# AndreasKing-Goks/ast-sac

Hardware: AMD Instinct MI355X
Metric: batched env-steps/sec (two-ship AST) (higher is better)
Workload: dtype f64

## Files before the change

### ast_sac_amd/build_hash.py

```python
import hashlib
import os

_HERE = os.path.dirname(os.path.abspath(__file__))
_ROOT = os.path.dirname(_HERE)

SOURCES = {
    "shipsim": ["ast_sac_amd/csrc/shipsim_kernels.hip", "ast_sac_amd/csrc/shipsim_c2_pipe.hip",
                "ast_sac_amd/csrc/shipsim_types.hpp", "ast_sac_amd/csrc/shipsim_device.hpp",
                "ast_sac_amd/csrc/shipsim_state.hpp", "ast_sac_amd/csrc/shipsim_sbmpc.hpp",
                "ast_sac_amd/csrc/shipsim_diag.hpp", "ast_sac_amd/csrc/shipsim_config_host.hpp",
                "ast_sac_amd/csrc/shipsim_weather_host.hpp", "ast_sac_amd/csrc/shipsim_launch_host.hpp",
                "ast_sac_amd/csrc/shipsim_state_host.hpp", "include/shipsim.h",
                "ast_sac_amd/csrc/shipsim_resample.hip", "ast_sac_amd/csrc/shipsim_resample_host.hpp",
                "ast_sac_amd/csrc/shipsim_archive.hip", "ast_sac_amd/csrc/shipsim_archive_host.hpp",
                "ast_sac_amd/csrc/shipsim_grouping_host.hpp", "ast_sac_amd/csrc/shipsim_sbmpc_nominal.hpp",
                "ast_sac_amd/csrc/shipsim_tree.hip", "ast_sac_amd/csrc/shipsim_tree_host.hpp",
                "ast_sac_amd/csrc/shipsim_weather.hip"],
    "sacfused": ["ast_sac_amd/csrc/sac_kernels.hip", "include/sac_fused.h"],
}


HIPFLAGS = ["-O3", "--offload-arch=gfx950", "-ffp-contract=off", "-fPIC", "-shared", "-std=c++17"]
LIB_FLAGS = {"shipsim": ["-mllvm", "-amdgpu-sched-strategy=max-ilp", "-mllvm", "-amdgpu-use-amdgpu-trackers"],
             "sacfused": []}
OBJECTS = {"sacfused": [("ast_sac_amd/csrc/sac_kernels.hip", ["-DSACF_TU=1", "-mllvm", "-amdgpu-sched-strategy=max-ilp"]),
                        ("ast_sac_amd/csrc/sac_kernels.hip", ["-DSACF_TU=2"])],
           "shipsim": [("ast_sac_amd/csrc/shipsim_kernels.hip", ["-mllvm", "-disable-machine-licm"]),
                       ("ast_sac_amd/csrc/shipsim_c2_pipe.hip", []),
                       ("ast_sac_amd/csrc/shipsim_resample.hip", []),
                       ("ast_sac_amd/csrc/shipsim_archive.hip", []),
                       ("ast_sac_amd/csrc/shipsim_tree.hip", []),
                       ("ast_sac_amd/csrc/shipsim_weather.hip", [])]}


def lib_objects(lib):
    return [(src, LIB_FLAGS[lib] + extra) for src, extra in OBJECTS[lib]]


def lib_flag_sets(lib):
    return [flags for _, flags in lib_objects(lib)]
# ... 18 lines not shown
```

### ast_sac_amd/csrc/shipsim_device.hpp

```cpp
#pragma once
#include <hip/hip_runtime.h>
#include <stdint.h>

#include <type_traits>

#include "shipsim.h"
#include "shipsim_diag.hpp"
#include "shipsim_types.hpp"

namespace shipsim {

__device__ __forceinline__ double div_rcp(double d) {
  double r = __builtin_amdgcn_rcp(d);
  r = fma(r, fma(-d, r, 1.0), r);
  return fma(r, fma(-d, r, 1.0), r);
}
__device__ __forceinline__ double div_by(double n, double d, double y) {
  const double q0 = n * y;
  const double rem = fma(-d, q0, n);
  return __builtin_amdgcn_div_fixup(fma(rem, y, q0), d, n);
}

struct LaneWeather {
  double vc_n, vc_e, wind_speed, wind_sin, wind_cos;
};
constexpr int kWeatherCols = 5;
enum { WX_WIND_SPEED = 0, WX_WIND_SIN = 1, WX_WIND_COS = 2, WX_VC_N = 3, WX_VC_E = 4 };

struct AccI {
  int32_t a;
  __device__ __forceinline__ void set(int32_t x) { asm("v_accvgpr_write_b32 %0, %1" : "=a"(a) : "v"(x)); }
// ... 87 lines not shown

template <int CTRL>
__device__ __forceinline__ double dpp_d(double x) {
  int lo = __double2loint(x), hi = __double2hiint(x);
  lo = __builtin_amdgcn_mov_dpp(lo, CTRL, 0xF, 0xF, false);
  hi = __builtin_amdgcn_mov_dpp(hi, CTRL, 0xF, 0xF, false);
  return __hiloint2double(hi, lo);
}
template <int CTRL>
__device__ __forceinline__ int dpp_i(int x) { return __builtin_amdgcn_mov_dpp(x, CTRL, 0xF, 0xF, false); }
constexpr int kDppRowBcast = 0x150;
constexpr int kDppRowRor4 = 0x124;
constexpr int kDppRowRor8 = 0x128;
constexpr int kDppQuadXor2 = 0x4E;
constexpr int kDppQuadXor1 = 0xB1;

__device__ __forceinline__ double pair_swap(double x) {
  int lo = __double2loint(x), hi = __double2hiint(x);
  lo = __builtin_amdgcn_mov_dpp(lo, 0xB1, 0xF, 0xF, false);
  hi = __builtin_amdgcn_mov_dpp(hi, 0xB1, 0xF, 0xF, false);
  return __hiloint2double(hi, lo);
}
__device__ __forceinline__ int pair_swap_i(int x) { return __builtin_amdgcn_mov_dpp(x, 0xB1, 0xF, 0xF, false); }

struct Deriv {
  double dn, de, dyaw, du, dv, dr, domega;
};

__device__ __forceinline__ double sub_pair_swap(double x) {
  int lo = __double2loint(x), hi = __double2hiint(x);
  lo = __builtin_amdgcn_mov_dpp(lo, 0x4E, 0xF, 0xF, false);
  hi = __builtin_amdgcn_mov_dpp(hi, 0x4E, 0xF, 0xF, false);
  return __hiloint2double(hi, lo);
}

template <bool PAIRED>
__device__ __forceinline__ void sincos2(double a, double b, bool odd, double& sa, double& ca, double& sb, double& cb) {
  if (PAIRED) {
    double s_, c_;
    sincos(odd ? b : a, &s_, &c_);
    const double so = sub_pair_swap(s_), co = sub_pair_swap(c_);
    sa = odd ? so : s_; ca = odd ? co : c_;
    sb = odd ? s_ : so; cb = odd ? c_ : co;
  } else {
    sincos(a, &sa, &ca);
    sincos(b, &sb, &cb);
// ... 361 lines not shown
```

### ast_sac_amd/csrc/shipsim_kernels.hip

```cpp
#include <hip/hip_runtime.h>

#include <math.h>
#include <stdarg.h>
#include <stdio.h>
#include <stdlib.h>
#include <string.h>

#include <new>
#include <type_traits>

#include "shipsim.h"
#include "shipsim_device.hpp"
#include "shipsim_state.hpp"
#include "shipsim_config_host.hpp"
#include "shipsim_launch_host.hpp"
#include "shipsim_weather_host.hpp"
#include "shipsim_grouping_host.hpp"
#include "shipsim_state_host.hpp"
#include "shipsim_archive_host.hpp"

#include "shipsim_diag.hpp"

#ifndef SHIPSIM_SB_NOMINAL
#define SHIPSIM_SB_NOMINAL 3
#endif

using namespace shipsim;
static_assert(kWeatherCols == weather_host::kCols && WX_WIND_SPEED == weather_host::kWindSpeed &&
                  WX_WIND_SIN == weather_host::kWindSin && WX_WIND_COS == weather_host::kWindCos &&
                  WX_VC_N == weather_host::kCurrentN && WX_VC_E == weather_host::kCurrentE,
              "the weather array's columns: device and host agree");

struct Traj {
  double* ship;
  double* env;
  double* fuel;
  int32_t* len;
  int32_t cap;
  __device__ __forceinline__ double* ship_row(int q, int t) const {
    return (t >= 0 && t < cap) ? ship + ((size_t)q * cap + t) * SHIPSIM_TRAJ_SHIP_COLS : nullptr;
  }
  __device__ __forceinline__ double* env_row(int e, int t) const {
    return (env && t >= 0 && t < cap) ? env + ((size_t)e * cap + t) * SHIPSIM_TRAJ_ENV_COLS : nullptr;
  }
};

template <bool DETAILED, bool REC, bool PRE = false, class PP>
__device__ __forceinline__ void control_and_store(const ShipConst& c, const PP& P, Ship& s,
                                                  const double* __restrict__ rn, const double* __restrict__ re,
                                                  double offset, double speed_factor, double mach_dt,
                                                  int simple_collav_flag ,
                                                  bool imminent, double* row, double* fuel, double& ctrl_out,
                                                  double& rudder_out, double pre_q = 0.0, double pre_e = 0.0) {
  const double N = s.n, E = s.e, H = s.yaw, U = s.u;
  double href;
  if constexpr (PRE) {
    double q = pre_q, e_ct = pre_e;
    if (next_wpt_advance(c, s, N, E)) {
      s.next_wpt += 1;
      load_segment(s, rn, re);
      q = los_q(c, s, N, E, e_ct);
    }
    s.e_ct = e_ct;
    href = s.seg_alpha + atan(los_windup(c, s, q));
  } else {
    if (next_wpt_advance(c, s, N, E)) {
      s.next_wpt += 1;
      load_segment(s, rn, re);
    }
    href = los_guidance(c, s, N, E);
  }
  double rudder = heading_ctrl(c, s, href + offset, H, P.dt, c.rcp_dt);
  double ctrl = speed_ctrl(c, s, c.desired_speed * speed_factor, U, P.dt, DETAILED, c.rcp_dt);
  if (simple_collav_flag && imminent) {
    ctrl *= 0.5;
    ctrl = py_min(py_max(ctrl, 0.0), 1.1);
    rudder += (simple_collav_flag == 1 ? -15.0 : 15.0) * (kPi / 180.0);
    rudder = py_min(py_max(rudder, -c.max_rudder), c.max_rudder);
  }
  s.log_rudder = rudder;
  s.log_ect = s.e_ct;
  s.log_n = N;
  s.log_e = E;
  s.log_thrust = DETAILED ? (c.thrust_coeff * s.omega * fabs(s.omega)) / 1000 : ctrl;
  if (REC) {
    if (DETAILED) fuel_consumption(c, ctrl, mach_dt, fuel);
    if (row) {
// ... 20 lines not shown
                                                      double* fuel = nullptr, bool odd = false, double wsin = 0.0,
                                                      double wcos = 1.0) {
  double ctrl, rudder;
  control_and_store<DETAILED, REC>(c, P, s, rn, re, offset, speed_factor, mach_dt, simple_collav_flag, imminent, row,
                                   fuel, ctrl, rudder);
  Deriv d = differentials<PAIRED, ALGW>(c, P, s, ctrl, rudder, DETAILED, odd, wsin, wcos);
  integrate(s, d, P.dt, mach_dt, DETAILED);
}

template <bool DETAILED, bool REC = false, bool PRE = false, class W = Params, class PP>
__device__ __forceinline__ void control_and_integrate_sc(const ShipConst& c, const PP& P, const W& wx, Ship& s,
                                                         const double* __restrict__ rn,
                                                         const double* __restrict__ re, double offset,
                                                         double speed_factor, double mach_dt, int simple_collav_flag,
                                                         bool imminent, double* row, double* fuel, double& sy,
                                                         double& cy, double pre_q = 0.0, double pre_e = 0.0) {
  double ctrl, rudder;
  control_and_store<DETAILED, REC, PRE>(c, P, s, rn, re, offset, speed_factor, mach_dt, simple_collav_flag, imminent,
                                        row, fuel, ctrl, rudder, pre_q, pre_e);
  Deriv d = differentials_sc(c, wx, s, ctrl, rudder, DETAILED, sy, cy);
  integrate(s, d, P.dt, mach_dt, DETAILED);
  sincos(s.yaw, &sy, &cy);
}
template <bool DETAILED, bool REC = false, bool PRE = false, class W = Params, class PP>
__device__ __forceinline__ void control_and_integrate_sc(const ShipConst& c, const PP& P, const W& wx, Ship& s,
                                                         const double* __restrict__ rn,
                                                         const double* __restrict__ re, double offset,
                                                         double speed_factor, double mach_dt, double n1, double e1,
                                                         double& sy, double& cy, double pre_q, double pre_e) {
  double ctrl, rudder;
  control_and_store<DETAILED, REC, PRE>(c, P, s, rn, re, offset, speed_factor, mach_dt, 0, false, nullptr, nullptr, ctrl,
                                        rudder, pre_q, pre_e);
  Deriv d = differentials_sc(c, wx, s, ctrl, rudder, DETAILED, sy, cy);
  integrate(s, d, n1, e1, P.dt, mach_dt, DETAILED);
  sincos(s.yaw, &sy, &cy);
}

__device__ __forceinline__ void record_last(const Traj& T, int q, int t, double time, double time_list) {
  double* row = T.ship_row(q, t);
  const double* prev = T.ship_row(q, t - 1);
  if (!row || !prev) return;
  for (int k = 0; k < SHIPSIM_TRAJ_SHIP_COLS; ++k) row[k] = prev[k];
  row[SHIPSIM_TS_TIME] = time;
  row[SHIPSIM_TS_REPEAT] = 1.0;
  row[SHIPSIM_TS_TIME_LIST] = time_list;
}

#include "shipsim_sbmpc.hpp"

__global__ void init_kernel(const Params P, DevState S, ConstBuf K) {
  const int q = blockIdx.x * blockDim.x + threadIdx.x;
  const int nq = P.n_envs * P.n_ships;
  if (q >= nq) return;
  const int ship = q % P.n_ships;
  const int env = q / P.n_ships;
  const ShipConst& c = K.ships()[ship];
  Ship s;
  s.n = c.init_n; s.e = c.init_e; s.yaw = c.init_yaw; s.u = c.init_u; s.v = c.init_v; s.r = c.init_r;
// ... 540 lines not shown
  const Traj& T = A0.T;
  const int max_ticks = A0.max_ticks;
  static_assert(!(REC && CHAIN), "trajectory recording runs the per-decision step only");
  static_assert(SLOTS == 2 || (LPE == 16 && !REC && COLLAV != SHIPSIM_COLLAV_SIMPLE), "multi-obstacle layout");
  static_assert(!WX || (DETAILED && !REC && COLLAV != SHIPSIM_COLLAV_SIMPLE), "per-env weather kernels");
  constexpr int NSUB = LPE / SLOTS;
  static_assert(NSUB >= 1 && 8 % NSUB == 0, "sub-lanes per ship must divide 8 (grid_part shares)");
  static_assert(LPE >= 2 && (LPE & (LPE - 1)) == 0 && LPE <= 16, "LPE must be a power of two in [2, 16]");
  constexpr bool SIMPLE = COLLAV == SHIPSIM_COLLAV_SIMPLE;
  constexpr bool OPQ = LPE != 16 || POLICY || SLOTS > 2;
  constexpr bool OPM = POLICY && SLOTS > 2;
  constexpr bool RC_PAR = DETAILED && LPE == 16 && !REC && SLOTS == 2 && (MODE == 1 || MODE == 2) && !SIMPLE;
  constexpr bool EARLY_MAP = RC_PAR;
  constexpr bool FLAT = RC_PAR;
  static_assert(!FLAT || (LPE == 16 && SLOTS == 2), "the flat tick: env = one DPP row, going per env");
#ifndef SHIPSIM_LANE_MATH
#define SHIPSIM_LANE_MATH 7
#endif
  constexpr bool LM_POST = FLAT && (SHIPSIM_LANE_MATH & 1);
  constexpr bool LM_OUT = FLAT && (SHIPSIM_LANE_MATH & 2);
  constexpr bool LM_REQ = FLAT && (SHIPSIM_LANE_MATH & 4);
  constexpr bool SB_NOM = LM_REQ && COLLAV == SHIPSIM_COLLAV_SBMPC && (SHIPSIM_SB_NOMINAL & 1);
  constexpr bool SB_NOM_ALG = SB_NOM && (SHIPSIM_SB_NOMINAL & 2);
  using flag_t = std::conditional_t<OPM, int, bool>;
#define OPM_GET(x) (OPM ? (decltype(x))opaque_v((int)(x)) : (x))
#define OPM_SET(x, v)                                  \
  {                                                    \
    if constexpr (OPM) x = opaque_v((v) ? 1 : 0);      \
    else x = (v);                                      \
  }
  __shared__ ShipConst lds_sc[SHIPSIM_MAX_SHIPS];
  __shared__ EdgeX lds_edges[SHIPSIM_MAX_VERTS];
  __shared__ Edge lds_edges_raw[SHIPSIM_MAX_VERTS];
  __shared__ PolyBox lds_boxes[SHIPSIM_MAX_POLYS];
  constexpr int kPolRows = SLOTS > 2 ? kPolMultiRows : kPolMaxRows;
  static_assert(SLOTS == 2 || 64 / LPE <= kPolMultiRows, "a policy pass serves every env of the wave");
  __shared__ float lds_pol[POLICY ? kPolRows * kPolMaxHidden : 1];
  __shared__ RewardTerm lds_rterm[8];
  if constexpr (diag::kPoisonLds) {
    diag::poison_lds(lds_sc, sizeof(lds_sc)); diag::poison_lds(lds_edges, sizeof(lds_edges));
    diag::poison_lds(lds_edges_raw, sizeof(lds_edges_raw)); diag::poison_lds(lds_boxes, sizeof(lds_boxes));
    __syncthreads();
  }
  const ShipConst* SC = stage_consts(K, lds_sc, P.n_ships, P.dt);
  for (int i = threadIdx.x; i < K.n_edges; i += blockDim.x) {
    const Edge ed = K.edges()[i];
// ... 252 lines not shown
          OPM_SET(want, true);
        }
      }
      float a_log;
      const float sa = chain_action(want, a_log);
      if (OPM_GET(want)) decision_prologue(sa, a_log);
    }
  };

  {
    const flag_t want = OPM ? (flag_t)opaque_v((running && (dflags & DF_AWAITING)) ? 1 : 0)
                            : (flag_t)(running && (dflags & DF_AWAITING));
    if (CHAIN) {
      float a_log;
      const float sa = chain_action(want, a_log);
      if (OPM_GET(want)) decision_prologue(sa, a_log);
    } else if (want) {
      decision_prologue(A0.action[envc], A0.action[envc]);
    }
  }

  int g_cell = -2, g_flag = GRID_MIXED;
  uint64_t g_mask = 0;
  int going = opaque_if<OPQ>((running && !ready && (budget <= 0 || ticks < budget)) ? 1 : 0);
  PT_DECL;
  for (;;) {
  while (__any(opaque_if<OPQ>(going)) && !(CHAIN && __any(opaque_if<OPQ>(ready) && opaque_if<OPQ>(running)))) {
    const StepArgs& A = step_args();
    const Params& P = A.P;
    const ConstBuf& K = A.K;
    const Traj& T = A.T;
    const auto& PT = regs_or<RC_PAR>(rc_par, P);
    const auto& KT = regs_or<RC_PAR>(rc_par, K);
    const int lie_t = opaque_if<OPQ>(lie);
    const int ship = lie_t % SLOTS;
    const int sub = lie_t / SLOTS;
    const bool is_test = ship == 0;
    const int nsh = (SLOTS == 2) ? 2 : P.n_ships;
    const bool ghost = (SLOTS > 2) && ship >= nsh;
    const int shipc = ghost ? nsh - 1 : ship;
    const bool is_obs1 = shipc == 1;
    (void)ghost;
    SHIPSIM_LANE_CHECK(LPE, 7);
    const double pn = pair_swap(s.n), pe = pair_swap(s.e);
    double sf = 1.0, off = 0.0;
    constexpr bool LOS_PRE = COLLAV == SHIPSIM_COLLAV_SBMPC && SLOTS == 2;
// ... 166 lines not shown
          if (cc >= 0) {
            g_mask = grid_share(K, cc, sub, NSUB);
            g_flag = (int)K.grid_flag[cc];
          }
        }
      }
      if (!is_test && s.stop) {
        if (REC && sub == 0) record_last(T, qc, rec_t, s.time, s.time + PT.dt);
        s.time = s.time + PT.dt;
        s.time = s.time + PT.dt;
      } else {
        const double prev_log_n = s.log_n, prev_log_e = s.log_e;
        const double U = s.u;
        bool imminent = false;
        if (SIMPLE && is_test) {
          float dn = st4[0] - st4[2], de = st4[1] - st4[3];
          imminent = (dn * dn + de * de) < 9000000.0f;
        }
        SHIPSIM_SHIP_CHECK(LPE, SLOTS, 6);
        if constexpr (RC_PAR) {
          const LaneWeather wxr = {PT.vc_n, PT.vc_e, PT.wind_speed, PT.wind_sin, PT.wind_cos};
          static_assert(EARLY_MAP == RC_PAR, "the step and the new position were formed at the top of the ship tick");
          const TickStep pd = {ep_dt};
          control_and_integrate_sc<DETAILED, REC, LOS_PRE>(c, pd, wxr, s, rn, re, -off, sf, mach_dt, ep_n, ep_e, sy, cy,
                                                           los_pre_q, los_pre_e);
        } else {
          control_and_integrate_sc<DETAILED, REC, LOS_PRE>(c, P, weather_of(P, lw), s, rn, re, -off, sf, mach_dt,
                                                           (SIMPLE && is_test) ? 1 : 0, imminent,
                                                           (REC && sub == 0) ? T.ship_row(qc, rec_t) : nullptr, fuel, sy,
                                                           cy, los_pre_q, los_pre_e);
        }
        my_speed_out = U;
        if (is_obs1) {
          double tn = s.log_n - prev_log_n, te = s.log_e - prev_log_e;
          if constexpr (LM_POST) dtravel2 = tn * tn + te * te;
          else dtravel = sqrt(tn * tn + te * te);
          dtime = PT.dt;
        }
      }
    }
    PT_MARK(1);
    double d2 = INFINITY;
    bool gr = false;
    if (FLAT || going) {
      int cc;
      if constexpr (EARLY_MAP) {
        cc = g_cell;
      } else {
// ... 119 lines not shown
      ns[3] = (float)On; ns[4] = (float)Oe; ns[5] = (float)Oyaw; ns[6] = (float)Ospeed; ns[7] = (float)Oect;
      if (SIMPLE) { st4[0] = ns[0]; st4[1] = ns[1]; st4[2] = ns[3]; st4[3] = ns[4]; }
      const bool is_collision = ((Tn - Cn) * (Tn - Cn) + (Te - Ce) * (Te - Ce)) < 2500.0;
      const bool is_tg = Tf & XF_GROUND, is_og = Of & XF_GROUND;
      const bool is_tnav = fabs(Tect) > 3000;
      const bool is_onav = (travel_dist > PT.AB_seg * 2) || (travel_time > INFINITY) || (fabs(Oect) > 500);
      double dx = Cn - Tn, dy = Ce - Te;
      double dist;
      if constexpr (LM_POST) dist = lm_dist;
      else dist = sqrt(dx * dx + dy * dy);
      const bool enc_ok = !overtaking_sector(dx, dy, dist, Tsh, Tch, Th);
      const double xv[5] = {dist, Tground, fabs(Tect), Oground, fabs(Oect)};
      const double tg[5] = {0.0, 0.0, 3000.0, 0.0, 500.0};
      const double of[5] = {200000000.0, 175000.0, 1250000.0, 50000.0, 12500.0};
      double ex[5];
      if (LPE >= 8) {
        const int j = opaque_v(lie) & 7;
        double xj;
        if constexpr (SLOTS == 2)
          xj = (j == 0) ? dist : (j < 3) ? Tground : fabs(Tect);
        else
          xj = (j == 0) ? xv[0] : (j == 1) ? xv[1] : (j == 2) ? xv[2] : (j == 3) ? xv[3] : xv[4];
        const RewardTerm to = lds_rterm[j];
        const double ej = exp(div_by(-((xj - to.t) * (xj - to.t)), to.o, to.y));
        ex[0] = env_lane_d<LPE, reward_lane<SLOTS>(0)>(ej, env_lane0);
        ex[1] = env_lane_d<LPE, reward_lane<SLOTS>(1)>(ej, env_lane0);
        ex[2] = env_lane_d<LPE, reward_lane<SLOTS>(2)>(ej, env_lane0);
        ex[3] = env_lane_d<LPE, reward_lane<SLOTS>(3)>(ej, env_lane0);
        ex[4] = env_lane_d<LPE, reward_lane<SLOTS>(4)>(ej, env_lane0);
      } else {
#pragma unroll
        for (int k = 0; k < 5; ++k) ex[k] = exp(-((xv[k] - tg[k]) * (xv[k] - tg[k])) / of[k]);
      }
      double r0 = (dist < 10000 && enc_ok) ? ((xv[0] < 0.0) ? 1.0 : ex[0]) : 0.0;
      double r1 = (Tground <= 1000) ? ((xv[1] < 0.0) ? 1.0 : ex[1]) : 0.0;
      double r2 = (xv[2] < 3000.0) ? ex[2] : 1.0;
      double r3 = (Oground <= 1000) ? -((xv[3] < 0.0) ? 1.0 : ex[3]) : 0.0;
      double r4 = -((xv[4] < 500.0) ? ex[4] : 1.0);
      double r = (r0 + ((((0.0 + r1) + r2) + r3) + r4)) / 5;
      if (is_collision || is_tg || is_tnav || is_og || is_onav) {
        const double reward = r + acc;
        double o = 0;
        const bool cond[5] = {is_collision, is_tg, is_tnav, is_og, is_onav};
        const double mult[5] = {10.0, 5.0, 5.0, -2.5, -2.5};
        for (int i = 0; i < 5; ++i) {
          if (acc > 0 && cond[i]) o += reward * mult[i];
          else if (acc < 0 && cond[i]) o += reward * -mult[i];
// ... 516 lines not shown
    out[(size_t)i * 3 + 1] = active ? cb : 0.0;
    out[(size_t)i * 3 + 2] = active ? 1.0 : 0.0;
  }
}

__global__ __launch_bounds__(64) void sbmpc_nominal_kernel(int n, double tf, double dt, const double* __restrict__ in,
                                                           int32_t* __restrict__ flag_out) {
  const int i = blockIdx.x * 64 + threadIdx.x;
  if (i >= n) return;
  const double* r = in + (size_t)i * SHIPSIM_SBMPC_IN;
  SbIn q;
  q.p_last = r[0]; q.chi_last = r[1]; q.u_d = r[2]; q.chi_d = r[3];
  q.os_x = r[4]; q.os_y = r[5]; q.os_v = r[8];
  q.ob_x = r[10]; q.ob_y = r[11]; q.ob_psi = r[12]; q.ob_u = r[13]; q.ob_v = r[14];
  sb_set_heading_trig(q);
  q.obs_l = r[15]; q.obs_w = r[16];
  double seg_sin, seg_cos, a;
  sbmpc_nominal_split_course(q.chi_d, seg_sin, seg_cos, a);
  const int n_samp = (int)(tf / dt);
  flag_out[i] = (sbmpc_nominal_holds(q, n_samp, dt).holds ? 1 : 0) |
                (sbmpc_nominal_holds_seg(q, seg_sin, seg_cos, a, n_samp, dt).holds ? 2 : 0);
}

template <int NOB>
__global__ __launch_bounds__(64) void sbmpc_multi_eval_kernel(int n, int n_obs, int n_samp, double dt,
                                                              const double* __restrict__ in, double* __restrict__ out) {
  const int i = blockIdx.x * 64 + threadIdx.x;
  const bool valid = i < n;
  const double* r = in + (size_t)(valid ? i : 0) * SHIPSIM_SBMPC_MULTI_IN;
  SbMulti<NOB> q;
  q.p_last = r[0]; q.chi_last = r[1]; q.u_d = r[2]; q.chi_d = r[3];
  q.os_x = r[4]; q.os_y = r[5]; q.os_v = r[8];
  bool active = false;
#pragma unroll
  for (int k = 0; k < NOB; ++k) {
    const double* o = r + 10 + 7 * k;
    q.ob_x[k] = o[0]; q.ob_y[k] = o[1]; q.ob_psi[k] = o[2]; q.ob_u[k] = o[3]; q.ob_v[k] = o[4];
    q.obs_l[k] = o[5]; q.obs_w[k] = o[6];
    const double d0 = o[0] - q.os_x, d1 = o[1] - q.os_y;
    if (k < n_obs) active = active || sqrt_lt(d0 * d0 + d1 * d1, 2000.0);
  }
  active = valid && active;
  double pb = 1.0, cb = 0.0;
  sbmpc_cooperative_multi<NOB>(active, q, n_obs, n_samp, dt, pb, cb);
  if (valid) {
    out[(size_t)i * 3 + 0] = active ? pb : 1.0;
// ... 871 lines not shown
  h->wx_moved = 1;
  shipsim_weather_gather_launch(h->stream, h->wx_dev, h->wx_stage, src_env, h->P.n_envs, h->P.n_envs, true);
  HIPCHK(h, hipGetLastError());
  HIPCHK(h, hipMemcpyAsync(h->wx_dev, h->wx_stage, (size_t)weather_host::store_bytes(h->P.n_envs),
                           hipMemcpyDeviceToDevice, h->stream));
  return SHIPSIM_OK;
}

int shipsim_sbmpc_eval(int32_t n, double tf, double dt, const double* in, double* out, void* stream) {
  if (n < 0 || (n > 0 && (!in || !out)) || !(dt > 0) || tf / dt > 4096) return SHIPSIM_EINVAL;
  if (n == 0) return SHIPSIM_OK;
  hipLaunchKernelGGL(sbmpc_eval_kernel, dim3((n + 63) / 64), dim3(64), 0, (hipStream_t)stream, n, tf, dt, in, out);
  return hipGetLastError() == hipSuccess ? SHIPSIM_OK : SHIPSIM_EHIP;
}

int shipsim_sbmpc_nominal(int32_t n, double tf, double dt, const double* in, int32_t* flag_out, void* stream) {
  if (n < 0 || (n > 0 && (!in || !flag_out)) || !(dt > 0) || tf / dt > 4096) return SHIPSIM_EINVAL;
  if (n == 0) return SHIPSIM_OK;
  hipLaunchKernelGGL(sbmpc_nominal_kernel, dim3((n + 63) / 64), dim3(64), 0, (hipStream_t)stream, n, tf, dt, in,
                     flag_out);
  return hipGetLastError() == hipSuccess ? SHIPSIM_OK : SHIPSIM_EHIP;
}

int shipsim_sbmpc_eval_multi(int32_t n, int32_t n_obs, double tf, double dt, const double* in, double* out,
                             void* stream) {
  if (n < 0 || n_obs < 1 || n_obs > SHIPSIM_MAX_OBS || (n > 0 && (!in || !out)) || !(dt > 0) || tf / dt > 4096)
    return SHIPSIM_EINVAL;
  if (n == 0) return SHIPSIM_OK;
  constexpr int kNob4 = launch_host::sbmpc_nob(4), kNob8 = launch_host::sbmpc_nob(8);
  static_assert(kNob4 < kNob8 && kNob8 == SHIPSIM_MAX_OBS, "every n_obs <= SHIPSIM_MAX_OBS has an instantiation");
  const bool wide = launch_host::sbmpc_nob(launch_host::ship_slots(1 + n_obs)) > kNob4;
  const dim3 grid((n + 63) / 64), block(64);
  const int n_samp = (int)(tf / dt);
  if (wide)
    hipLaunchKernelGGL(sbmpc_multi_eval_kernel<kNob8>, grid, block, 0, (hipStream_t)stream, n, n_obs, n_samp, dt, in,
                       out);
  else
    hipLaunchKernelGGL(sbmpc_multi_eval_kernel<kNob4>, grid, block, 0, (hipStream_t)stream, n, n_obs, n_samp, dt, in,
                       out);
  return hipGetLastError() == hipSuccess ? SHIPSIM_OK : SHIPSIM_EHIP;
}

int shipsim_div_check(int32_t n, const double* num, const double* den, double* fast, double* ref, void* stream) {
  if (n < 0 || (n > 0 && (!num || !den || !fast || !ref))) return SHIPSIM_EINVAL;
  if (n == 0) return SHIPSIM_OK;
  hipLaunchKernelGGL(div_check_kernel, dim3((n + 255) / 256), dim3(256), 0, (hipStream_t)stream, n, num, den, fast,
// ... 50 lines not shown
```

### ast_sac_amd/shipsim.py

```python
import ctypes as C
import os

import numpy as np
import torch

from . import shipsim_abi as abi

_HERE = os.path.dirname(os.path.abspath(__file__))
LIB_PATH = os.environ.get("SHIPSIM_LIB") or os.path.join(_HERE, "lib", "libshipsim.so")

_lib = None


class ShipSimError(RuntimeError):
    pass


class ShipSimNonFiniteError(ShipSimError):
    """shipsim_synchronize: env decisions ended on a NaN/Inf ship state (SHIPSIM_EV_NONFINITE)."""


def load_library(path=LIB_PATH):
    global _lib
    if _lib is not None:
# ... 30 lines not shown
    L.shipsim_set_stream_tail.argtypes = [P, C.c_int32]
    for name, argtypes in (("shipsim_div_check", [C.c_int32, P, P, P, P, P]),
                           ("shipsim_diag_lane_faults", [P]),
                           ("shipsim_run_policy", [P, P, P, C.c_int32, C.c_int32, C.c_int32, C.c_uint64, P, C.c_int32,
                                                   C.c_int32, P, P, P, P, P, C.c_int32, P]),
                           ("shipsim_sbmpc_eval_multi", [C.c_int32, C.c_int32, C.c_double, C.c_double, P, P, P]),
                           ("shipsim_set_weather", [P, P, P, P, P]),
                           ("shipsim_get_weather", [P, P, P, P, P]),
                           ("shipsim_state_bytes", [P]),
                           ("shipsim_snapshot", [P, P, C.c_int64]),
                           ("shipsim_restore", [P, P, C.c_int64]),
                           ("shipsim_fork", [P, P, C.c_int64, P]),
                           ("shipsim_resample_workspace_bytes", [C.c_int32]),
                           ("shipsim_resample", [C.c_int32, P, P, C.c_uint64, P, C.c_int32, P, C.c_int64, P, P, P, P, P]),
                           ("shipsim_level_distance", [P, P]),
                           ("shipsim_archive_bytes", [P, C.c_int32]),
                           ("shipsim_archive_store", [P, P, C.c_int64, C.c_int32, P]),
                           ("shipsim_archive_load", [P, P, C.c_int64, C.c_int32, P]),
                           ("shipsim_archive_workspace_bytes", [C.c_int32]),
                           ("shipsim_archive_elect", [C.c_int32, C.c_int32, P, P, P, P, P, C.c_int64, P, P, P]),
                           ("shipsim_set_stream_grouping", [P, C.c_int32]),
                           ("shipsim_get_stream_grouping", [P, P]),
                           ("shipsim_sbmpc_nominal", [C.c_int32, C.c_double, C.c_double, P, P, P]),
                           ("shipsim_tree_bytes", [C.c_int32, C.c_int32]),
                           ("shipsim_tree_layout", [C.c_int32, C.c_int32, P]),
                           ("shipsim_tree_workspace_bytes", [C.c_int32, C.c_int32]),
                           ("shipsim_tree_init", [P, C.c_int64, C.c_int32, C.c_int32, P]),
                           ("shipsim_tree_select", [P, C.c_int64, C.c_int32, C.c_int32, C.c_int32, C.c_int32, C.c_int32,
                                                    C.c_int32, C.c_double, P, C.c_int64, P, P, P]),
                           ("shipsim_tree_expand", [P, C.c_int64, C.c_int32, C.c_int32, C.c_int32, P, P, P, P, C.c_int64,
                                                    P, P]),
                           ("shipsim_tree_backup", [P, C.c_int64, C.c_int32, C.c_int32, C.c_int32, P, P, P, P]),
                           ("shipsim_weather_bytes", [C.c_int32]),
                           ("shipsim_weather_store", [P, P, C.c_int64, C.c_int32, P]),
                           ("shipsim_weather_load", [P, P, C.c_int64, C.c_int32, P]),
                           ("shipsim_weather_fork", [P, P])):
        try:
            getattr(L, name).argtypes = argtypes
            if name in ("shipsim_state_bytes", "shipsim_resample_workspace_bytes", "shipsim_archive_bytes",
                        "shipsim_archive_workspace_bytes", "shipsim_tree_bytes", "shipsim_tree_workspace_bytes",
                        "shipsim_weather_bytes"):
                getattr(L, name).restype = C.c_int64
        except AttributeError:
            if "SHIPSIM_LIB" not in os.environ:
                raise
    if L.shipsim_abi_version() != abi.ABI_VERSION:
# ... 1 lines not shown
    from .build_hash import check_library
    try:
        check_library("shipsim", L.shipsim_build_info().decode(), path, explicit="SHIPSIM_LIB" in os.environ)
    except RuntimeError as e:
        raise ShipSimError(str(e)) from None
    _lib = L
    return L


EXPORTED_SYMBOLS = ("shipsim_abi_version", "shipsim_build_info", "shipsim_default_config", "shipsim_create",
                    "shipsim_destroy", "shipsim_last_error", "shipsim_num_envs", "shipsim_reset", "shipsim_step",
                    "shipsim_tick", "shipsim_get_state", "shipsim_set_state", "shipsim_synchronize",
                    "shipsim_set_trajectory", "shipsim_sbmpc_eval", "shipsim_legacy_step", "shipsim_run_table",
                    "shipsim_nonfinite_count", "shipsim_lanes_per_env", "shipsim_set_stream",
                    "shipsim_run_policy", "shipsim_diag_lane_faults", "shipsim_set_stream_tail", "shipsim_div_check",
                    "shipsim_sbmpc_eval_multi", "shipsim_set_weather", "shipsim_get_weather",
                    "shipsim_state_bytes", "shipsim_snapshot", "shipsim_restore", "shipsim_fork",
                    "shipsim_resample_workspace_bytes", "shipsim_resample", "shipsim_level_distance",
                    "shipsim_archive_bytes", "shipsim_archive_store", "shipsim_archive_load",
                    "shipsim_archive_workspace_bytes", "shipsim_archive_elect", "shipsim_set_stream_grouping",
                    "shipsim_get_stream_grouping", "shipsim_sbmpc_nominal", "shipsim_tree_bytes", "shipsim_tree_layout",
                    "shipsim_tree_workspace_bytes", "shipsim_tree_init", "shipsim_tree_select", "shipsim_tree_expand",
                    "shipsim_tree_backup", "shipsim_weather_bytes", "shipsim_weather_store", "shipsim_weather_load",
                    "shipsim_weather_fork")


class Snapshot:

    __slots__ = ("data", "kind", "n_envs", "n_ships", "build", "weather")

    def __init__(self, data, kind, n_envs, n_ships, build, weather=None):
        self.data, self.kind, self.n_envs, self.n_ships, self.build = data, int(kind), int(n_envs), int(n_ships), build
        self.weather = weather

    def clone(self):
        return Snapshot(self.data.clone(), self.kind, self.n_envs, self.n_ships, self.build,
                        None if self.weather is None else self.weather.clone())


class StateArchive:

    def __init__(self, sim, n_cells, weather=False):
        n_cells = int(n_cells)
        if not 1 <= n_cells <= abi.ARCHIVE_MAX_CELLS:
            raise ShipSimError(f"archive: n_cells must be in 1..{abi.ARCHIVE_MAX_CELLS}, not {n_cells}")
        if weather and not sim._weather_on:
            raise ShipSimError("archive: weather=True needs a handle with per-env weather in force (set_weather)")
# ... 457 lines not shown
    L = load_library()
    x = torch.as_tensor(requests, dtype=torch.float64, device=device).contiguous()
    if x.dim() != 2 or x.shape[1] != abi.SBMPC_IN:
        raise ShipSimError(f"requests must be (n, {abi.SBMPC_IN})")
    out = torch.empty((x.shape[0], 3), dtype=torch.float64, device=x.device)
    stream = torch.cuda.current_stream(x.device)
    rc = L.shipsim_sbmpc_eval(int(x.shape[0]), float(tf), float(dt), _ptr(x), _ptr(out), C.c_void_p(stream.cuda_stream))
    if rc:
        raise ShipSimError(f"shipsim_sbmpc_eval failed ({rc})")
    return out


def sbmpc_nominal(requests, tf=1000.0, dt=20.0, device="cuda"):
    L = load_library()
    x = torch.as_tensor(requests, dtype=torch.float64, device=device).contiguous()
    if x.dim() != 2 or x.shape[1] != abi.SBMPC_IN:
        raise ShipSimError(f"requests must be (n, {abi.SBMPC_IN})")
    out = torch.zeros(x.shape[0], dtype=torch.int32, device=x.device)
    stream = torch.cuda.current_stream(x.device)
    rc = L.shipsim_sbmpc_nominal(int(x.shape[0]), float(tf), float(dt), _ptr(x), _ptr(out),
                                 C.c_void_p(stream.cuda_stream))
    if rc:
        raise ShipSimError(f"shipsim_sbmpc_nominal failed ({rc})")
    return out


def sbmpc_eval_multi(requests, n_obs, tf=1000.0, dt=20.0, device="cuda"):
    L = load_library()
    x = torch.as_tensor(requests, dtype=torch.float64, device=device).contiguous()
    if x.dim() != 2 or x.shape[1] != abi.SBMPC_MULTI_IN:
        raise ShipSimError(f"requests must be (n, {abi.SBMPC_MULTI_IN})")
    out = torch.empty((x.shape[0], 3), dtype=torch.float64, device=x.device)
    stream = torch.cuda.current_stream(x.device)
    rc = L.shipsim_sbmpc_eval_multi(int(x.shape[0]), int(n_obs), float(tf), float(dt), _ptr(x), _ptr(out),
                                    C.c_void_p(stream.cuda_stream))
    if rc:
        if rc != -1:
            why = "the launch failed"
        elif not 1 <= int(n_obs) <= abi.MAX_OBS:
            why = f"n_obs {int(n_obs)} must be 1..{abi.MAX_OBS}"
        else:
            why = f"bad argument (tf {float(tf)}, dt {float(dt)}: dt > 0 and tf / dt <= 4096)"
        raise ShipSimError(f"shipsim_sbmpc_eval_multi failed ({rc}): {why}")
    return out


# ... 180 lines not shown
```

### include/shipsim.h

```cpp
#ifndef SHIPSIM_H
#define SHIPSIM_H

#include <stdint.h>

#ifdef __cplusplus
extern "C" {
#endif

#define SHIPSIM_ABI_VERSION 12

#define SHIPSIM_MAX_ROUTE 16
#define SHIPSIM_MAX_POLYS 16
#define SHIPSIM_MAX_VERTS 128
#define SHIPSIM_MAX_OBS 4
#define SHIPSIM_MAX_SHIPS (1 + SHIPSIM_MAX_OBS)

#define SHIPSIM_OK 0
#define SHIPSIM_EINVAL -1
#define SHIPSIM_EHIP -2
#define SHIPSIM_ESTATE -3
#define SHIPSIM_ENOMEM -4
#define SHIPSIM_ENONFINITE -5

#define SHIPSIM_KIND_SINGLE 0
// ... 246 lines not shown
#define SHIPSIM_TS_NEXT_WPT 17
#define SHIPSIM_TS_REPEAT 18
#define SHIPSIM_TS_TIME_LIST 19
#define SHIPSIM_TRAJ_ENV_COLS 8
#define SHIPSIM_TE_R_COLLISION 0
#define SHIPSIM_TE_R_TEST_GROUNDING 1
#define SHIPSIM_TE_R_TEST_NAV 2
#define SHIPSIM_TE_R_OBS_GROUNDING 3
#define SHIPSIM_TE_R_OBS_NAV 4
#define SHIPSIM_TE_R_TOTAL 5
#define SHIPSIM_TE_BITS 6
#define SHIPSIM_TE_FLAGS 7
#define SHIPSIM_TE_FLAG_COLLISION 1
#define SHIPSIM_TE_FLAG_IMMINENT 2

int shipsim_set_trajectory(shipsim_handle* h, double* ship_rows, double* env_rows, int32_t capacity,
                           int32_t* lengths);

#define SHIPSIM_SBMPC_IN 17
int shipsim_sbmpc_eval(int32_t n, double tf, double dt, const double* in, double* out, void* stream);

int shipsim_sbmpc_nominal(int32_t n, double tf, double dt, const double* in, int32_t* flag_out, void* stream);

#define SHIPSIM_SBMPC_MULTI_IN (10 + 7 * SHIPSIM_MAX_OBS)
int shipsim_sbmpc_eval_multi(int32_t n, int32_t n_obs, double tf, double dt, const double* in, double* out,
                             void* stream);

int shipsim_div_check(int32_t n, const double* num, const double* den, double* fast, double* ref, void* stream);

#define SHIPSIM_DECLOG_COLS 23
#define SHIPSIM_DL_REWARD 0
#define SHIPSIM_DL_EVENTS 1
#define SHIPSIM_DL_DONE 2
#define SHIPSIM_DL_EPISODE 3
#define SHIPSIM_DL_DECISION 4
#define SHIPSIM_DL_TICKS 5
#define SHIPSIM_DL_OBS 6
#define SHIPSIM_DL_ACTION 14
#define SHIPSIM_DL_OBS0 15
int shipsim_run_table(shipsim_handle* h, const float* table, int32_t n_eps, int32_t n_dec, int32_t max_ticks,
                      int32_t* ep_idx, int32_t* dec_idx, int32_t* ticks_out, int32_t* decisions_out, double* log,
                      int32_t log_cap, int32_t* log_len);

int shipsim_run_policy(shipsim_handle* h, const float* policy, const float* w2t, int32_t obs_dim, int32_t hidden,
                       int32_t deterministic, uint64_t seed, const int64_t* counter, int32_t n_dec,
                       int32_t max_ticks, int32_t* ep_idx, int32_t* dec_idx, int32_t* ticks_out,
// ... 39 lines not shown
```

Measured before the change: 1.167 billion.

## Inline custom sincos/atan/exp with DPP-broadcast coefficient table in ship tick

Adds hand-written double-precision sincos, atan and exp kernels (Cody-Waite reduction plus polynomials) and uses them for the yaw sincos, LOS atan and reward exp in the flat SBMPC tick path. The default mode keeps polynomial coefficients spread across a 16-lane row in registers and broadcasts them with DPP instead of materialising literal constants, with a wave-row vote that falls back to libm sincos for large arguments. This aims to cut the instruction and scalar-register cost of the libm calls. It risks accuracy differences from libm, DPP latency, and extra VGPR pressure. A test kernel and API are added to compare the implementations.

```diff
diff --git a/ast_sac_amd/build_hash.py b/ast_sac_amd/build_hash.py
--- a/ast_sac_amd/build_hash.py
+++ b/ast_sac_amd/build_hash.py
@@ -15,7 +15,7 @@
                 "ast_sac_amd/csrc/shipsim_archive.hip", "ast_sac_amd/csrc/shipsim_archive_host.hpp",
                 "ast_sac_amd/csrc/shipsim_grouping_host.hpp", "ast_sac_amd/csrc/shipsim_sbmpc_nominal.hpp",
                 "ast_sac_amd/csrc/shipsim_tree.hip", "ast_sac_amd/csrc/shipsim_tree_host.hpp",
-                "ast_sac_amd/csrc/shipsim_weather.hip"],
+                "ast_sac_amd/csrc/shipsim_weather.hip", "ast_sac_amd/csrc/shipsim_tickmath.hpp"],
     "sacfused": ["ast_sac_amd/csrc/sac_kernels.hip", "include/sac_fused.h"],
 }
 
diff --git a/ast_sac_amd/csrc/shipsim_device.hpp b/ast_sac_amd/csrc/shipsim_device.hpp
--- a/ast_sac_amd/csrc/shipsim_device.hpp
+++ b/ast_sac_amd/csrc/shipsim_device.hpp
@@ -7,6 +7,7 @@
 #include "shipsim.h"
 #include "shipsim_diag.hpp"
 #include "shipsim_types.hpp"
+#include "shipsim_tickmath.hpp"
 
 namespace shipsim {
 
@@ -140,6 +141,67 @@
   return __hiloint2double(hi, lo);
 }
 __device__ __forceinline__ int pair_swap_i(int x) { return __builtin_amdgcn_mov_dpp(x, 0xB1, 0xF, 0xF, false); }
+
+struct TmRow {
+  static constexpr int kEvenPairs = (tickmath::kExp0 + 7) / 8, kPairs = kEvenPairs + 1;
+  static_assert(tickmath::kCount - tickmath::kExp0 <= 16, "the exp entries fit one row");
+  double t[kPairs];
+  __device__ __forceinline__ void load(int lane_in_row) {
+#pragma unroll
+    for (int p = 0; p < kEvenPairs; ++p) {
+      const int i = p * 8 + (lane_in_row >> 1);
+      t[p] = tickmath::tm_entry(i < tickmath::kExp0 ? i : -1);
+    }
+    t[kEvenPairs] = tickmath::tm_entry(tickmath::kExp0 + lane_in_row);
+  }
+  template <int I>
+  __device__ __forceinline__ double k() const {
+    static_assert(I >= 0 && I < tickmath::kCount, "tickmath table index");
+    constexpr int pair = I < tickmath::kExp0 ? I / 8 : kEvenPairs;
+    constexpr int lane = I < tickmath::kExp0 ? 2 * (I % 8) : I - tickmath::kExp0;
+    return __builtin_amdgcn_mov_dpp(t[pair], kDppRowBcast + lane, 0xF, 0xF, true);
+  }
+  template <int I>
+  __device__ __forceinline__ double kd(double dead) const {
+    static_assert(I >= 0 && I < tickmath::kCount, "tickmath table index");
+    constexpr int pair = I < tickmath::kExp0 ? I / 8 : kEvenPairs;
+    constexpr int lane = I < tickmath::kExp0 ? 2 * (I % 8) : I - tickmath::kExp0;
+    return __builtin_amdgcn_update_dpp(dead, t[pair], kDppRowBcast + lane, 0xF, 0xF, false);
+  }
+};
+
+template <int BITS>
+struct TickMath {
+  TmRow row;
+  int row_lane0;
+  __device__ __forceinline__ void sincos_yaw(double x, double* s, double* c) const {
+    if constexpr ((BITS & 2) == 0) {
+      sincos(x, s, c);
+    } else {
+      bool ok = tickmath::tm_sincos_small_ok(x);
+      if constexpr (BITS & 4) {
+        const uint64_t out = __ballot(!ok);
+        ok = ((uint32_t)(out >> row_lane0) & 0xFFFFu) == 0u;
+      }
+      if (ok) {
+        if constexpr (BITS & 4) tickmath::tm_sincos(x, row, s, c);
+        else tickmath::tm_sincos(x, tickmath::TmLiteral(), s, c);
+      } else {
+        sincos(x, s, c);
+      }
+    }
+  }
+  __device__ __forceinline__ double atan_los(double x) const {
+    if constexpr (BITS & 4) return tickmath::tm_atan(x, row);
+    else if constexpr (BITS & 1) return tickmath::tm_atan(x, tickmath::TmLiteral());
+    else return atan(x);
+  }
+  __device__ __forceinline__ double exp_reward(double x) const {
+    if constexpr (BITS & 4) return tickmath::tm_exp(x, row);
+    else if constexpr (BITS & 1) return tickmath::tm_exp(x, tickmath::TmLiteral());
+    else return exp(x);
+  }
+};
 
 struct Deriv {
   double dn, de, dyaw, du, dv, dr, domega;
diff --git a/ast_sac_amd/csrc/shipsim_kernels.hip b/ast_sac_amd/csrc/shipsim_kernels.hip
--- a/ast_sac_amd/csrc/shipsim_kernels.hip
+++ b/ast_sac_amd/csrc/shipsim_kernels.hip
@@ -24,6 +24,9 @@
 #ifndef SHIPSIM_SB_NOMINAL
 #define SHIPSIM_SB_NOMINAL 3
 #endif
+#ifndef SHIPSIM_TICK_MATH
+#define SHIPSIM_TICK_MATH 7
+#endif
 
 using namespace shipsim;
 static_assert(kWeatherCols == weather_host::kCols && WX_WIND_SPEED == weather_host::kWindSpeed &&
@@ -45,13 +48,14 @@
   }
 };
 
-template <bool DETAILED, bool REC, bool PRE = false, class PP>
+template <bool DETAILED, bool REC, bool PRE = false, class PP, class TM = TickMath<0>>
 __device__ __forceinline__ void control_and_store(const ShipConst& c, const PP& P, Ship& s,
                                                   const double* __restrict__ rn, const double* __restrict__ re,
                                                   double offset, double speed_factor, double mach_dt,
                                                   int simple_collav_flag ,
                                                   bool imminent, double* row, double* fuel, double& ctrl_out,
-                                                  double& rudder_out, double pre_q = 0.0, double pre_e = 0.0) {
+                                                  double& rudder_out, double pre_q = 0.0, double pre_e = 0.0,
+                                                  const TM& tm = TM()) {
   const double N = s.n, E = s.e, H = s.yaw, U = s.u;
   double href;
   if constexpr (PRE) {
@@ -62,7 +66,7 @@
       q = los_q(c, s, N, E, e_ct);
     }
     s.e_ct = e_ct;
-    href = s.seg_alpha + atan(los_windup(c, s, q));
+    href = s.seg_alpha + tm.atan_los(los_windup(c, s, q));
   } else {
     if (next_wpt_advance(c, s, N, E)) {
       s.next_wpt += 1;
@@ -129,18 +133,19 @@
   integrate(s, d, P.dt, mach_dt, DETAILED);
   sincos(s.yaw, &sy, &cy);
 }
-template <bool DETAILED, bool REC = false, bool PRE = false, class W = Params, class PP>
+template <bool DETAILED, bool REC = false, bool PRE = false, class W = Params, class PP, class TM = TickMath<0>>
 __device__ __forceinline__ void control_and_integrate_sc(const ShipConst& c, const PP& P, const W& wx, Ship& s,
                                                          const double* __restrict__ rn,
                                                          const double* __restrict__ re, double offset,
                                                          double speed_factor, double mach_dt, double n1, double e1,
-                                                         double& sy, double& cy, double pre_q, double pre_e) {
+                                                         double& sy, double& cy, double pre_q, double pre_e,
+                                                         const TM& tm = TM()) {
   double ctrl, rudder;
   control_and_store<DETAILED, REC, PRE>(c, P, s, rn, re, offset, speed_factor, mach_dt, 0, false, nullptr, nullptr, ctrl,
-                                        rudder, pre_q, pre_e);
+                                        rudder, pre_q, pre_e, tm);
   Deriv d = differentials_sc(c, wx, s, ctrl, rudder, DETAILED, sy, cy);
   integrate(s, d, n1, e1, P.dt, mach_dt, DETAILED);
-  sincos(s.yaw, &sy, &cy);
+  tm.sincos_yaw(s.yaw, &sy, &cy);
 }
 
 __device__ __forceinline__ void record_last(const Traj& T, int q, int t, double time, double time_list) {
@@ -727,6 +732,8 @@
   constexpr bool LM_REQ = FLAT && (SHIPSIM_LANE_MATH & 4);
   constexpr bool SB_NOM = LM_REQ && COLLAV == SHIPSIM_COLLAV_SBMPC && (SHIPSIM_SB_NOMINAL & 1);
   constexpr bool SB_NOM_ALG = SB_NOM && (SHIPSIM_SB_NOMINAL & 2);
+  constexpr bool TM_KERNEL = FLAT && COLLAV == SHIPSIM_COLLAV_SBMPC && !POLICY;
+  constexpr int TMB = TM_KERNEL ? ((SHIPSIM_TICK_MATH & 4) ? 7 : (SHIPSIM_TICK_MATH & 3)) : 0;
   using flag_t = std::conditional_t<OPM, int, bool>;
 #define OPM_GET(x) (OPM ? (decltype(x))opaque_v((int)(x)) : (x))
 #define OPM_SET(x, v)                                  \
@@ -1025,6 +1032,9 @@
 
   int g_cell = -2, g_flag = GRID_MIXED;
   uint64_t g_mask = 0;
+  TickMath<TMB> tmath;
+  tmath.row_lane0 = env_lane0;
+  if constexpr (TMB & 4) tmath.row.load(lie);
   int going = opaque_if<OPQ>((running && !ready && (budget <= 0 || ticks < budget)) ? 1 : 0);
   PT_DECL;
   for (;;) {
@@ -1237,8 +1247,10 @@
           const LaneWeather wxr = {PT.vc_n, PT.vc_e, PT.wind_speed, PT.wind_sin, PT.wind_cos};
           static_assert(EARLY_MAP == RC_PAR, "the step and the new position were formed at the top of the ship tick");
           const TickStep pd = {ep_dt};
+          if constexpr (TMB & 4)
+            SHIPSIM_INDEX_CHECK(((__builtin_amdgcn_read_exec() >> env_lane0) & 0x5555u) == 0x5555u, 14);
           control_and_integrate_sc<DETAILED, REC, LOS_PRE>(c, pd, wxr, s, rn, re, -off, sf, mach_dt, ep_n, ep_e, sy, cy,
-                                                           los_pre_q, los_pre_e);
+                                                           los_pre_q, los_pre_e, tmath);
         } else {
           control_and_integrate_sc<DETAILED, REC, LOS_PRE>(c, P, weather_of(P, lw), s, rn, re, -off, sf, mach_dt,
                                                            (SIMPLE && is_test) ? 1 : 0, imminent,
@@ -1404,7 +1416,8 @@
         else
           xj = (j == 0) ? xv[0] : (j == 1) ? xv[1] : (j == 2) ? xv[2] : (j == 3) ? xv[3] : xv[4];
         const RewardTerm to = lds_rterm[j];
-        const double ej = exp(div_by(-((xj - to.t) * (xj - to.t)), to.o, to.y));
+        if constexpr (TMB & 4) SHIPSIM_LANE_CHECK(LPE, 15);
+        const double ej = tmath.exp_reward(div_by(-((xj - to.t) * (xj - to.t)), to.o, to.y));
         ex[0] = env_lane_d<LPE, reward_lane<SLOTS>(0)>(ej, env_lane0);
         ex[1] = env_lane_d<LPE, reward_lane<SLOTS>(1)>(ej, env_lane0);
         ex[2] = env_lane_d<LPE, reward_lane<SLOTS>(2)>(ej, env_lane0);
@@ -1967,6 +1980,36 @@
                 (sbmpc_nominal_holds_seg(q, seg_sin, seg_cos, a, n_samp, dt).holds ? 2 : 0);
 }
 
+__global__ __launch_bounds__(64) void tickmath_eval_kernel(int fn, int n, const double* __restrict__ x,
+                                                           double* __restrict__ out) {
+  const int i = blockIdx.x * 64 + threadIdx.x;
+  const double a = x[i < n ? i : n - 1];
+  const int lane = (int)(threadIdx.x & 63);
+  TickMath<3> lit;
+  lit.row_lane0 = lane & ~15;
+  TickMath<7> row;
+  row.row_lane0 = lane & ~15;
+  row.row.load(lane & 15);
+  double v[6] = {0, 0, 0, 0, 0, 0};
+  if (fn == 0) {
+    sincos(a, &v[0], &v[1]);
+    lit.sincos_yaw(a, &v[2], &v[3]);
+    row.sincos_yaw(a, &v[4], &v[5]);
+  } else if (fn == 1) {
+    v[0] = atan(a);
+    v[2] = lit.atan_los(a);
+    v[4] = row.atan_los(a);
+  } else {
+    v[0] = exp(a);
+    v[2] = lit.exp_reward(a);
+    v[4] = row.exp_reward(a);
+  }
+  if (i < n) {
+#pragma unroll
+    for (int k = 0; k < 6; ++k) out[(size_t)i * 6 + k] = v[k];
+  }
+}
+
 template <int NOB>
 __global__ __launch_bounds__(64) void sbmpc_multi_eval_kernel(int n, int n_obs, int n_samp, double dt,
                                                               const double* __restrict__ in, double* __restrict__ out) {
@@ -2884,6 +2927,13 @@
   return hipGetLastError() == hipSuccess ? SHIPSIM_OK : SHIPSIM_EHIP;
 }
 
+int shipsim_tickmath_eval(int32_t fn, int32_t n, const double* in, double* out, void* stream) {
+  if (fn < 0 || fn > 2 || n < 0 || (n > 0 && (!in || !out))) return SHIPSIM_EINVAL;
+  if (n == 0) return SHIPSIM_OK;
+  hipLaunchKernelGGL(tickmath_eval_kernel, dim3((n + 63) / 64), dim3(64), 0, (hipStream_t)stream, fn, n, in, out);
+  return hipGetLastError() == hipSuccess ? SHIPSIM_OK : SHIPSIM_EHIP;
+}
+
 int shipsim_sbmpc_eval_multi(int32_t n, int32_t n_obs, double tf, double dt, const double* in, double* out,
                              void* stream) {
   if (n < 0 || n_obs < 1 || n_obs > SHIPSIM_MAX_OBS || (n > 0 && (!in || !out)) || !(dt > 0) || tf / dt > 4096)
diff --git a/ast_sac_amd/csrc/shipsim_tickmath.hpp b/ast_sac_amd/csrc/shipsim_tickmath.hpp
--- /dev/null
+++ b/ast_sac_amd/csrc/shipsim_tickmath.hpp
@@ -0,0 +1,216 @@
+#pragma once
+#include <math.h>
+#include <stdint.h>
+
+#include "shipsim_types.hpp"
+
+namespace shipsim {
+namespace tickmath {
+
+constexpr int kSinCos0 = 0, kAtan0 = 16, kExp0 = 38, kCount = 51;
+constexpr double kTm[kCount] = {
+    0x1.45f306dc9c883p-1,
+    -0x1.921fb54442d18p+0,
+    -0x1.1a62633145c00p-54,
+    -0x1.b839a252049c0p-104,
+    -0x1.907db46cc5e42p-37,
+    0x1.1eeb69037ab78p-29,
+    -0x1.27e4fa17f65f6p-22,
+    0x1.a01a019f4ec90p-16,
+    -0x1.6c16c16c16967p-10,
+    0x1.5555555555555p-5,
+    0x1.5e0b2f9a43bb8p-33,
+    -0x1.ae600b42fdfa7p-26,
+    0x1.71de3796cde01p-19,
+    -0x1.a01a019e83e5cp-13,
+    0x1.1111111110bb3p-7,
+    -0x1.5555555555555p-3,
+    0x1.ba404b5e68a13p-17,
+    -0x1.3e260bd3237f4p-13,
+    0x1.b2bb069efb384p-11,
+    -0x1.7952daf56de9bp-9,
+    0x1.d6d43a595c56fp-8,
+    -0x1.c6ea4a57d9582p-7,
+    0x1.67e295f08b19fp-6,
+    -0x1.e9ae6fc27006ap-6,
+    0x1.2c15b5711927ap-5,
+    -0x1.59976e82d3ff0p-5,
+    0x1.82d5d6ef28734p-5,
+    -0x1.ae5ce6a214619p-5,
+    0x1.e1bb48427b883p-5,
+    -0x1.110e48b207f05p-4,
+    0x1.3b13657b87036p-4,
+    -0x1.745d119378e4fp-4,
+    0x1.c71c717e1913cp-4,
+    -0x1.2492492376b7dp-3,
+    0x1.99999999952ccp-3,
+    -0x1.5555555555523p-2,
+    0x1.dd9ad336a0500p-1,
+    0x1.af154eeb562d6p+0,
+    0x1.71547652b82fep+0,
+    0x1.62e42fefa39efp-1,
+    0x1.abc9e3b39803fp-56,
+    0x1.ade156a5dcb37p-26,
+    0x1.28af3fca7ab0cp-22,
+    0x1.71dee623fde64p-19,
+    0x1.a01997c89e6b0p-16,
+    0x1.a01a014761f6ep-13,
+    0x1.6c16c1852b7b0p-10,
+    0x1.1111111122322p-7,
+    0x1.55555555502a1p-5,
+    0x1.5555555555511p-3,
+    0x1.000000000000bp-1,
+};
+
+SHIPSIM_HD double tm_entry(int i) { return (i >= 0 && i < kCount) ? kTm[i] : 0.0; }
+
+struct TmLiteral {
+  template <int I>
+  SHIPSIM_HD double k() const {
+    static_assert(I >= 0 && I < kCount, "tickmath table index");
+    return kTm[I];
+  }
+  template <int I>
+  SHIPSIM_HD double kd(double dead) const {
+    (void)dead;
+    return k<I>();
+  }
+};
+
+SHIPSIM_HD uint64_t tm_bits(double x) {
+  uint64_t u;
+  __builtin_memcpy(&u, &x, 8);
+  return u;
+}
+SHIPSIM_HD double tm_from_bits(uint64_t u) {
+  double x;
+  __builtin_memcpy(&x, &u, 8);
+  return x;
+}
+SHIPSIM_HD int tm_to_int(double y) {
+#ifdef __HIP_DEVICE_COMPILE__
+  return (int)y;
+#else
+  return (y >= -2147483648.0 && y <= 2147483647.0) ? (int)y : 0;
+#endif
+}
+
+SHIPSIM_HD bool tm_sincos_small_ok(double x) { return fabs(x) < 0x1.0p+30; }
+
+template <class K>
+SHIPSIM_HD void tm_sincos(double x, const K& T, double* sp, double* cp) {
+  constexpr int B = kSinCos0;
+  const double ax = fabs(x);
+  const double y = rint(ax * T.template k<B + 0>());
+  const double r4 = fma(y, T.template k<B + 1>(), ax);
+  const double r5 = fma(y, T.template k<B + 2>(), r4);
+  const double pm = -T.template k<B + 2>();
+  const double r6 = y * pm;
+  const double r8 = fma(y, pm, -r6);
+  const double r9 = r4 - r6;
+  const double r10 = r4 - r9;
+  const double r11 = r10 - r6;
+  const double r12 = r9 - r5;
+  const double r13 = r12 + r11;
+  const double r14 = r13 - r8;
+  const double r15 = fma(y, T.template k<B + 3>(), r14);
+  const double hi = r5 + r15;
+  const double r17 = hi - r5;
+  const double lo = r15 - r17;
+  const int q = tm_to_int(y) & 3;
+  const double x2 = hi * hi;
+  const double h = x2 * 0.5;
+  const double c5 = 1.0 - h;
+  const double c6 = 1.0 - c5;
+  const double c7 = c6 - h;
+  const double x4 = x2 * x2;
+  const double p0 = fma(x2, T.template kd<B + 4>(r12), T.template kd<B + 5>(r13));
+  const double p1 = fma(x2, p0, T.template kd<B + 6>(r14));
+  const double p2 = fma(x2, p1, T.template kd<B + 7>(p0));
+  const double p3 = fma(x2, p2, T.template kd<B + 8>(p1));
+  const double p = fma(x2, p3, T.template kd<B + 9>(p2));
+  const double nlo = -lo;
+  const double c15 = fma(hi, nlo, c7);
+  const double c16 = fma(x4, p, c15);
+  const double cc = c5 + c16;
+  const double s0 = fma(x2, T.template kd<B + 10>(r10), T.template kd<B + 11>(r11));
+  const double s1 = fma(x2, s0, T.template kd<B + 12>(r17));
+  const double s2 = fma(x2, s1, T.template kd<B + 13>(s0));
+  const double s = fma(x2, s2, T.template kd<B + 14>(s1));
+  const double x3n = hi * (-x2);
+  const double hl = lo * 0.5;
+  const double s25 = fma(x3n, s, hl);
+  const double s26 = fma(x2, s25, nlo);
+  const double s27 = fma(x3n, T.template kd<B + 15>(s2), s26);
+  const double ss = hi - s27;
+  const uint64_t flip = q > 1 ? 0x8000000000000000ull : 0ull;
+  const bool even = (q & 1) == 0;
+  const uint64_t sb = tm_bits(even ? ss : cc) ^ (tm_bits(x) & 0x8000000000000000ull) ^ flip;
+  const uint64_t cb = tm_bits(even ? cc : -ss) ^ flip;
+  *sp = tm_from_bits(sb);
+  *cp = tm_from_bits(cb);
+}
+
+template <class K>
+SHIPSIM_HD double tm_atan(double x, const K& T) {
+  constexpr int B = kAtan0;
+  const double ax = fabs(x);
+  const bool big = ax > 1.0;
+  const double rc = 1.0 / ax;
+  const double v = big ? rc : ax;
+  const double t = v * v;
+  const double q0 = fma(t, T.template kd<B + 0>(rc), T.template kd<B + 1>(ax));
+  const double q1 = fma(t, q0, T.template k<B + 2>());
+  const double q2 = fma(t, q1, T.template kd<B + 3>(q0));
+  const double q3 = fma(t, q2, T.template kd<B + 4>(q1));
+  const double q4 = fma(t, q3, T.template kd<B + 5>(q2));
+  const double q5 = fma(t, q4, T.template kd<B + 6>(q3));
+  const double q6 = fma(t, q5, T.template kd<B + 7>(q4));
+  const double q7 = fma(t, q6, T.template kd<B + 8>(q5));
+  const double q8 = fma(t, q7, T.template kd<B + 9>(q6));
+  const double q9 = fma(t, q8, T.template kd<B + 10>(q7));
+  const double q10 = fma(t, q9, T.template kd<B + 11>(q8));
+  const double q11 = fma(t, q10, T.template kd<B + 12>(q9));
+  const double q12 = fma(t, q11, T.template kd<B + 13>(q10));
+  const double q13 = fma(t, q12, T.template kd<B + 14>(q11));
+  const double q14 = fma(t, q13, T.template kd<B + 15>(q12));
+  const double q15 = fma(t, q14, T.template kd<B + 16>(q13));
+  const double q16 = fma(t, q15, T.template kd<B + 17>(q14));
+  const double q17 = fma(t, q16, T.template kd<B + 18>(q15));
+  const double q18 = fma(t, q17, T.template kd<B + 19>(q16));
+  const double p = q18;
+  const double tp = t * p;
+  const double red = fma(v, tp, v);
+  const double hi = fma(T.template k<B + 20>(), T.template k<B + 21>(), -red);
+  const double r = big ? hi : red;
+  return copysign(r, x);
+}
+
+template <class K>
+SHIPSIM_HD double tm_exp(double x, const K& T) {
+  constexpr int B = kExp0;
+  const double xl = x * T.template k<B + 0>();
+  const double n = rint(xl);
+  const double nn = -n;
+  const double r0 = fma(nn, T.template k<B + 1>(), x);
+  const double r = fma(nn, T.template kd<B + 2>(xl), r0);
+  const double e0 = fma(r, T.template kd<B + 3>(r0), T.template kd<B + 4>(nn));
+  const double e1 = fma(r, e0, T.template k<B + 5>());
+  const double e2 = fma(r, e1, T.template kd<B + 6>(e0));
+  const double e3 = fma(r, e2, T.template kd<B + 7>(e1));
+  const double e4 = fma(r, e3, T.template kd<B + 8>(e2));
+  const double e5 = fma(r, e4, T.template kd<B + 9>(e3));
+  const double e6 = fma(r, e5, T.template kd<B + 10>(e4));
+  const double e7 = fma(r, e6, T.template kd<B + 11>(e5));
+  const double e8 = fma(r, e7, T.template kd<B + 12>(e6));
+  double p = e8;
+  p = fma(r, p, 1.0);
+  p = fma(r, p, 1.0);
+  double z = ldexp(p, tm_to_int(n));
+  z = x > 1024.0 ? (double)INFINITY : z;
+  z = x < -1075.0 ? 0.0 : z;
+  return z;
+}
+
+}
+}
diff --git a/ast_sac_amd/shipsim.py b/ast_sac_amd/shipsim.py
--- a/ast_sac_amd/shipsim.py
+++ b/ast_sac_amd/shipsim.py
@@ -76,6 +76,7 @@
                            ("shipsim_set_stream_grouping", [P, C.c_int32]),
                            ("shipsim_get_stream_grouping", [P, P]),
                            ("shipsim_sbmpc_nominal", [C.c_int32, C.c_double, C.c_double, P, P, P]),
+                           ("shipsim_tickmath_eval", [C.c_int32, C.c_int32, P, P, P]),
                            ("shipsim_tree_bytes", [C.c_int32, C.c_int32]),
                            ("shipsim_tree_layout", [C.c_int32, C.c_int32, P]),
                            ("shipsim_tree_workspace_bytes", [C.c_int32, C.c_int32]),
@@ -123,7 +124,7 @@
                     "shipsim_get_stream_grouping", "shipsim_sbmpc_nominal", "shipsim_tree_bytes", "shipsim_tree_layout",
                     "shipsim_tree_workspace_bytes", "shipsim_tree_init", "shipsim_tree_select", "shipsim_tree_expand",
                     "shipsim_tree_backup", "shipsim_weather_bytes", "shipsim_weather_store", "shipsim_weather_load",
-                    "shipsim_weather_fork")
+                    "shipsim_weather_fork", "shipsim_tickmath_eval")
 
 
 class Snapshot:
@@ -627,6 +628,20 @@
                                  C.c_void_p(stream.cuda_stream))
     if rc:
         raise ShipSimError(f"shipsim_sbmpc_nominal failed ({rc})")
+    return out
+
+
+TICKMATH_FN = {"sincos": 0, "atan": 1, "exp": 2}
+
+
+def tickmath_eval(fn, x, device="cuda"):
+    L = load_library()
+    a = torch.as_tensor(x, dtype=torch.float64, device=device).contiguous().reshape(-1)
+    out = torch.zeros((a.shape[0], 3, 2), dtype=torch.float64, device=a.device)
+    stream = torch.cuda.current_stream(a.device)
+    rc = L.shipsim_tickmath_eval(TICKMATH_FN[fn], int(a.shape[0]), _ptr(a), _ptr(out), C.c_void_p(stream.cuda_stream))
+    if rc:
+        raise ShipSimError(f"shipsim_tickmath_eval failed ({rc})")
     return out
 
 
diff --git a/include/shipsim.h b/include/shipsim.h
--- a/include/shipsim.h
+++ b/include/shipsim.h
@@ -292,6 +292,8 @@
 
 int shipsim_sbmpc_nominal(int32_t n, double tf, double dt, const double* in, int32_t* flag_out, void* stream);
 
+int shipsim_tickmath_eval(int32_t fn, int32_t n, const double* in, double* out, void* stream);
+
 #define SHIPSIM_SBMPC_MULTI_IN (10 + 7 * SHIPSIM_MAX_OBS)
 int shipsim_sbmpc_eval_multi(int32_t n, int32_t n_obs, double tf, double dt, const double* in, double* out,
                              void* stream);
```

New measurement: 1.184 billion (median of 6 runs). +1.4%, better.
